# sagescherrytree/Project3-CUDA-Path-Tracer-2025

Measured on AMD Instinct MI355X. Metric: Mpaths/s (rays x bounces / s), 800x800 cornell depth 8, higher is better.
Workload: dtype f32; 1 GPU; cornell.json 800x800 depth 8, stream compaction on, sort off (BASELINE configs[1]); pipeline=fused, frames_per_pass=128, parallelism=single GPU

## Files before the change

### project3-cuda-path-tracer-2025_amd/csrc/pt_runtime.hip

```cpp
#include <dlfcn.h>
#include <hip/hip_runtime.h>
#include <hip/hip_ext.h>
#include <rccl/rccl.h>

#include <algorithm>
#include <cmath>
#include <condition_variable>
#include <mutex>
#include <thread>
#include <cstdarg>
#include <cstdlib>
#include <cstdio>
#include <cstring>
#include <string>
#include <vector>

#include "pt/pathtrace_abi.h"
#include "pt/pt_denoise.h"
#include "pt/pt_naive_mesh.h"
#include "pt_kernels.h"
#include "pt_denoise_kernels.h"
#include "pt_naive_mesh_kernels.h"
#include "trav_tree.h"

// ... 273 lines not shown
    }
    if (lds_geoms) stage_geoms(sc, s_dyn);
    PT_HOOK(STAGE_EXTRA, lds_geoms, sc, s_dyn);
    if (TIMING && active) {
        __builtin_amdgcn_s_waitcnt(0);
        uint64_t t = sec_clock();
        sec_add(SEC_LOAD, t - tc);
        sec_add(SEC_N_WAVES, 1);
        sec_add_lanes(SEC_N_LANES, p.rb > 0 ? 1 : 0);
    }
    bool live = active && p.rb > 0;
    constexpr bool MG = (VAR & VAR_MAT_GROUP) != 0;
    Hit h;
    if (MG) h = Hit{-1.f, mk(0.f, 0.f, 0.f), 0, -1, 0.f, 0.f};
    bool queued = false;
    float qt = 0.f;
    int qw = -1;
    f3 qs = mk(0.f, 0.f, 0.f);
    if (REDIST && lds_geoms) {
        if (VAR & VAR_BLOCK_REDIST)
            block_intersect<TIMING>(sc, s_geoms, live, p.o, p.d, reinterpret_cast<BlockLds*>(s_wave_isect - (tid >> 6)),
                                    qt, qw, qs);
        else
            wave_intersect<TIMING>(sc, s_geoms, live, p.o, p.d, s_wave_isect, qt, qw, qs);
    } else if (SPLIT && live) {
        prim_intersect_q<TIMING, FIRST && !TIMING>(sc, s_geoms, p.o, p.d, qt, qw, qs);
    }
    if (live) {
        if (SPLIT) {
            queued = bvh_root_needed(sc, p.o, p.d, qt);
            if (!queued) h = finish_hit<false>(sc, p.o, p.d, s_stack + tid, qt, qw, qs);
        } else if (REDIST && lds_geoms) {
            h = finish_hit<HAS_BVH, BVH_FAST>(sc, p.o, p.d, s_stack + tid, qt, qw, qs);
            PT_HOOK(DUP_HIT, HAS_BVH, BVH_FAST, sc, p.o, p.d, s_stack + tid, qt, qw, qs);
        } else {
            h = lds_geoms ? intersect_scene_q<HAS_BVH, TIMING, BVH_FAST, FIRST>(sc, s_geoms, p.o, p.d, s_stack + tid)
                          : intersect_scene<HAS_BVH, BVH_FAST>(sc, p.o, p.d, s_stack + tid);
        }
        if (!MG && !queued) {
            uint64_t ts = TIMING ? sec_clock() : 0;
            PT_HOOK(DUP_SHADE, (VAR & VAR_NO_TEX) == 0, sc, p, h, iter);
            shade_path<(VAR & VAR_NO_TEX) == 0>(sc, p, h, iter + p.slot, [&]() { return hit_attr(sc, h); });
            if (TIMING) {
                tc = sec_clock();
                sec_add(SEC_SHADE, tc - ts);
            }
        }
    }
    if (MG) {
        if (SPLIT) {
            int qi, unused;
            block_append<false>(queued, &ctl->qcnt[bounce][blockIdx.x & (NSEG - 1)][0], false, nullptr, qi, unused);
            qi += (blockIdx.x & (NSEG - 1)) * q.stride;
            if (queued) {
                queue_put(q, qi, p, qt, qw, qs);
                active = false;
                live = false;
                queued = false;
            }
        }
        const int key = live ? (h.t > 0.0f ? h.mat : 0) : MG_KEYS - 1;
        MatGroupLds* mg = reinterpret_cast<MatGroupLds*>(s_wave_isect - (tid >> 6));
        group_by_material<HAS_BVH, false>(key, mg, active, live, queued, p, h, qt, qw, qs);
        if (live) shade_path<(VAR & VAR_NO_TEX) == 0>(sc, p, h, iter + p.slot, [&]() { return hit_attr(sc, h); });
    }
    if (TIMING && active) tc = sec_clock();
    const bool surv = active && !queued && p.rb > 0;
    if (active && !queued && !surv) gather_into_image(image, sc, to_plane, p);
    const int lane = tid & 63;
    const int seg = blockIdx.x & (NSEG - 1);
    if (VAR & VAR_WAVE_ATOMIC) {
        const uint64_t m = __ballot(surv);
        if (m != 0) {
            int base = 0;
            if (lane == 0) base = atomicAdd(&ctl->cnt[bounce + 1][seg][0], __popcll(m));
            base = __shfl(base, 0);
            if (surv) store_path(out, seg * seg_stride + base + mbcnt(m), p);
        }
        if (!SPLIT) return;
        const uint64_t mq = __ballot(queued);
        if (mq != 0) {
            int base = 0;
            if (lane == 0) base = atomicAdd(&ctl->qcnt[bounce][seg][0], __popcll(mq));
            base = __shfl(base, 0);
            if (queued) {
                const int k = seg * q.stride + base + mbcnt(mq);
                queue_put(q, k, p, qt, qw, qs);
            }
        }
        return;
    }
    int si, qi;
    block_append<SPLIT>(surv, &ctl->cnt[bounce + 1][seg][0], queued, &ctl->qcnt[bounce][seg][0], si, qi);
    if (surv) store_path(out, seg * seg_stride + si, p);
    qi += seg * q.stride;
    if (SPLIT && queued) queue_put(q, qi, p, qt, qw, qs);
    if (TIMING && active) sec_add(SEC_STORE, sec_clock() - tc);
}

template <int VAR>
__global__ __launch_bounds__(BLOCK) void k_tail(SceneDev sc, PathBuf in, FrameCtl* ctl, float* __restrict__ image,
                                               int bounce, int seg_stride, int depth) {
    extern __shared__ float4 s_dyn[];
    __shared__ int s_cnt[BLOCK / 64];
    const int iter = ctl->iter;
    const bool to_plane = ctl->batch > 1 || ctl->plane != 0;
    int segoff[NSEG + 1];
    segoff[0] = 0;
#pragma unroll
    for (int s = 0; s < NSEG; ++s) segoff[s + 1] = segoff[s] + ctl->cnt[bounce][s][0];
    const int n = segoff[NSEG];
    const int block_start = blockIdx.x * BLOCK;
    if (block_start >= n) return;
    const int tid = threadIdx.x, lane = tid & 63;
    DevGeomHot* s_geoms = reinterpret_cast<DevGeomHot*>(s_dyn);
    BlockLds* s_block = reinterpret_cast<BlockLds*>(s_dyn + lds_geom_f4(sc));
    const int gid = block_start + tid;
    const bool active = gid < n;
    PathReg p;
    p.rb = 0;
    if (active) {
        int sl = 0;
#pragma unroll
        for (int k = 1; k < NSEG; ++k) sl += (gid >= segoff[k]) ? 1 : 0;
        int sofs = 0;
#pragma unroll
        for (int k = 1; k < NSEG; ++k) sofs = (sl == k) ? segoff[k] : sofs;
        p = load_path(in, sl * seg_stride + (gid - sofs));
    }
    stage_geoms(sc, s_dyn);
    const int seg = blockIdx.x & (NSEG - 1);
    for (int b = bounce; b < depth; ++b) {
        const bool live = active && p.rb > 0;
        float qt = 0.f;
        int qw = -1;
        f3 qs = mk(0.f, 0.f, 0.f);
        block_intersect<false>(sc, s_geoms, live, p.o, p.d, s_block, qt, qw, qs);
        if (live) {
            const Hit h = finish_hit<false>(sc, p.o, p.d, nullptr, qt, qw, qs);
            shade_path<(VAR & VAR_NO_TEX) == 0>(sc, p, h, iter + p.slot, [&]() { return hit_attr(sc, h); });
            if (p.rb <= 0) gather_into_image(image, sc, to_plane, p);
        }
        const bool surv = live && p.rb > 0;
        const uint64_t m = __ballot(surv);
        if (lane == 0) s_cnt[tid >> 6] = __popcll(m);
        __syncthreads();
        int tot = 0;
#pragma unroll
        for (int i = 0; i < BLOCK / 64; ++i) tot += s_cnt[i];
        if (tid == 0 && tot) atomicAdd(&ctl->cnt[b + 1][seg][0], tot);
        __syncthreads();
        if (tot == 0) break;
    }
}

#ifndef BVH_WAVES
#define BVH_WAVES 7
#endif

template <int VAR>
PT_DEV void bvh_finish_path(const SceneDev& sc, const QueueBuf& q, int qs, int iter, PathReg& p, const TravState& st) {
    float u = 0.f, v = 0.f;
    int tri = -1;
    const float tb = trav_result(st, u, v, tri);
    const float4 c = q.C[qs], d = q.D[qs];
    p.pix = __float_as_int(q.A[qs].w);
    p.rb = __float_as_int(q.B[qs].w);
    p.c = mk(c.x, c.y, c.z);
    const int cw = __float_as_int(c.w);
    p.slot = cw & 255;
    const int win = (cw >> 8) - 1;
    const Hit h = make_hit(sc, p.d, d.x, win, mk(d.y, d.z, d.w), tb, u, v, tri, sc.hot4);
    shade_path<(VAR & VAR_NO_TEX) == 0>(sc, p, h, iter + p.slot, [&]() { return hit_attr(sc, h); });
}
template <bool COUNT>
PT_DEV void bvh_count_ray(const TravState& st, float t_prim, int n_nodes) {
    if (COUNT) {
        sec_add_lanes(SEC_N_BVH_RAYS, 1);
        const bool hit = st.btri != 0x7fffffff && st.t_hit < t_prim;
        sec_add_lanes(SEC_N_BVH_HITS, hit ? 1 : 0);
        sec_add_lanes(SEC_N_MISS_NODES, hit ? 0 : n_nodes);
    }
}

PT_DEV bool tail_put(const TailBuf& t, int* ctr, int seg, int qs, const TravState& st, const int* s_stack) {
    const uint64_t m = __ballot(1);
    const int lead = __builtin_ctzll(m);
    int base = 0;
    if ((int)(threadIdx.x & 63) == lead) base = atomicAdd(ctr, __popcll(m));
    const int slot = __builtin_amdgcn_readlane(base, lead) + mbcnt(m);
    if (slot >= t.stride) return false;
    const int e = seg * t.stride + slot;
    t.node[e] = make_int2(qs, trav_saved_node(st));
    t.hit[e] = trav_saved_hit(st);
    for (int i = 0; i < min(st.sp, t.depth); ++i) t.stack[(size_t)i * t.cap + e] = s_stack[i * BLOCK];
    atomicAdd(ctr + 2, 1);
    atomicAdd(ctr + 3, st.sp);
    return true;
}

template <int VAR, bool QUAD>
__global__ __launch_bounds__(BLOCK, BVH_WAVES) void k_bvh_bounce(SceneDev sc, QueueBuf q, TailBuf tail, int defer,
                                                                 PathBuf out, FrameCtl* ctl, float* __restrict__ image,
                                                                 int bounce, int seg_stride) {
    extern __shared__ float4 s_dyn[];
    int segoff[NSEG + 1];
    segoff[0] = 0;
#pragma unroll
    for (int s = 0; s < NSEG; ++s) segoff[s + 1] = segoff[s] + ctl->qcnt[bounce][s][0];
    const int n = segoff[NSEG];
    const int block_start = blockIdx.x * BLOCK;
    if (block_start >= n) return;
    int* s_stack = reinterpret_cast<int*>(s_dyn);
    const int iter = ctl->iter;
    const bool to_plane = ctl->batch > 1 || ctl->plane != 0;
    const int tid = threadIdx.x;
    const int gid = block_start + tid;
    const int seg = blockIdx.x & (NSEG - 1);
    const bool active = gid < n;
    bool handed = false;
    const int qs = active ? segment_slot(segoff, gid, block_start, q.stride) : 0;
    PathReg p;
    p.rb = 0;
    if (active) {
        const float4 a = q.A[qs], b = q.B[qs];
        const float t_prim = q.D[qs].x;
        p.o = mk(a.x, a.y, a.z);
        p.d = mk(b.x, b.y, b.z);
        constexpr bool CNT = (VAR & VAR_SECTION_TIMING) != 0;
        int n_nodes = 0, n_tris = 0;
        TravState st;
        trav_begin(sc, st, p.o, p.d, t_prim);
        st.qs = qs;
        if (CNT) sec_add_lanes(SEC_N_ROOT_CULLED, st.cur < 0 ? 1 : 0);
        for (int d = defer;; d = 0) {
            trav_run<CNT, QUAD>(sc, st, s_stack + tid, d, n_nodes, n_tris);
            if (st.cur < 0) break;
            if (tail_put(tail, &ctl->qcnt[bounce][seg][1], seg, qs, st, s_stack + tid)) {
                handed = true;
                break;
            }
        }
        if (CNT) {
            sec_add_lanes(SEC_N_NODES, n_nodes);
            sec_add_lanes(SEC_N_TRIS, n_tris);
        }
        if (!handed) {
            bvh_count_ray<CNT>(st, t_prim, n_nodes);
            bvh_finish_path<VAR>(sc, q, qs, iter, p, st);
        }
    }
    const bool surv = active && !handed && p.rb > 0;
    if (active && !handed && !surv) gather_into_image(image, sc, to_plane, p);
    int si, unused;
    block_append<false>(surv, &ctl->cnt[bounce + 1][seg][0], false, nullptr, si, unused);
    if (surv) store_path(out, seg * seg_stride + si, p);
}

template <int VAR, bool QUAD>
__global__ __launch_bounds__(BLOCK, BVH_WAVES) void k_bvh_tail_trav(SceneDev sc, QueueBuf q, TailBuf t, FrameCtl* ctl,
                                                                    int bounce, int refill) {
    extern __shared__ float4 s_dyn[];
    int* s_stack = reinterpret_cast<int*>(s_dyn) + threadIdx.x;
    const int seg = blockIdx.x & (NSEG - 1);
    const int n = min(ctl->qcnt[bounce][seg][1], t.stride);
    if (n == 0) return;
    int next = 0;
    constexpr bool CNT = (VAR & VAR_SECTION_TIMING) != 0;
    int e = -1, qs = 0, n_nodes = 0, n_tris = 0, sp0 = 0;
    bool hit0 = false;
    TravState st;
    st.cur = -1;
    while (true) {
        const uint64_t idle = __ballot(e < 0);
        const int n_idle = __popcll(idle);
        if (next < n && (n_idle >= refill || n_idle == 64)) {
            const int lead = __builtin_ctzll(idle);
            int b0 = 0;
            if ((int)(threadIdx.x & 63) == lead) b0 = atomicAdd(&ctl->qcnt[bounce][seg][2], n_idle);
            next = __builtin_amdgcn_readlane(b0, lead);
            if (e < 0) {
                const int k = next + mbcnt(idle);
                if (k < n) {
                    e = seg * t.stride + k;
                    const int2 nd = t.node[e];
                    qs = nd.x;
                    const float4 a = q.A[qs], b = q.B[qs];
                    trav_resume(st, mk(a.x, a.y, a.z), mk(b.x, b.y, b.z), t.hit[e], nd.y, qs);
                    for (int i = 0; i < min(st.sp, sc.stack_lds); ++i) s_stack[i * BLOCK] = t.stack[(size_t)i * t.cap + e];
                    n_nodes = n_tris = 0;
                    if (CNT) {
                        sp0 = st.sp;
                        hit0 = st.btri != 0x7fffffff;
                    }
                }
            }
            next += n_idle;
        }
        const int lanes = __popcll(__ballot(e >= 0));
        if (lanes == 0) break;
        if (e >= 0) {
            if (CNT) {
                sec_add(SEC_N_BVH_WITERS, 1);
                sec_add(SEC_TAIL_LANES_HIST + (lanes - 1) / 4, 1);
            }
            trav_step<CNT, QUAD>(sc, st, s_stack, n_nodes, n_tris);
// ... 245 lines not shown
    __shared__ int h[MAXMAT];
    const int n = *n_ptr;
    const int tile = blockIdx.x, base = tile * STILE;
    for (int i = threadIdx.x; i < nkeys; i += BLOCK) h[i] = 0;
    __syncthreads();
    if (base < n) {
        for (int k = 0; k < STILE / BLOCK; ++k) {
            int idx = base + k * BLOCK + threadIdx.x;
            if (idx < n) atomicAdd(&h[keys[idx]], 1);
        }
    }
    __syncthreads();
    for (int i = threadIdx.x; i < nkeys; i += BLOCK) tile_hist[(size_t)tile * nkeys + i] = h[i];
}

__global__ __launch_bounds__(SCAN_THREADS) void k_sort_scan(int* tile_hist, const int* n_ptr, int nkeys) {
    __shared__ int s_part[SCAN_THREADS];
    const int n = *n_ptr;
    const int ntiles = (n + STILE - 1) / STILE;
    const int total = ntiles * nkeys;
    const int per = (total + SCAN_THREADS - 1) / SCAN_THREADS;
    const int tid = threadIdx.x;
    const int lo = min(total, tid * per), hi = min(total, lo + per);
    const int key0 = ntiles ? lo / ntiles : 0, t0 = lo - key0 * ntiles;
    int sum = 0;
    for (int f = lo, key = key0, t = t0; f < hi; ++f) {
        sum += tile_hist[(size_t)t * nkeys + key];
        if (++t == ntiles) { t = 0; ++key; }
    }
    s_part[tid] = sum;
    __syncthreads();
    for (int off = 1; off < SCAN_THREADS; off <<= 1) {
        const int v = tid >= off ? s_part[tid - off] : 0;
        __syncthreads();
        s_part[tid] += v;
        __syncthreads();
    }
    int run = tid ? s_part[tid - 1] : 0;
    for (int f = lo, key = key0, t = t0; f < hi; ++f) {
        const size_t at = (size_t)t * nkeys + key;
        const int c = tile_hist[at];
        tile_hist[at] = run;
        run += c;
        if (++t == ntiles) { t = 0; ++key; }
    }
}

__global__ __launch_bounds__(BLOCK) void k_sort_scatter(const int* __restrict__ keys, const int* n_ptr, int nkeys,
                                                        int key_bits, const int* tile_off, int* perm) {
    __shared__ int run[MAXMAT];
    __shared__ int wcnt[BLOCK / 64][MAXMAT];
    const int n = *n_ptr;
    const int tile = blockIdx.x, base = tile * STILE;
    if (base >= n) return;
    const int tid = threadIdx.x, w = tid >> 6;
    for (int i = tid; i < nkeys; i += BLOCK) run[i] = 0;
    __syncthreads();
    for (int k = 0; k < STILE / BLOCK; ++k) {
        int idx = base + k * BLOCK + tid;
        bool valid = idx < n;
        int key = valid ? keys[idx] : 0;
        uint64_t peers = __ballot(valid);
        for (int b = 0; b < key_bits; ++b) {
            uint64_t bb = __ballot(valid && ((key >> b) & 1));
            peers &= ((key >> b) & 1) ? bb : ~bb;
        }
        for (int i = tid; i < (BLOCK / 64) * MAXMAT; i += BLOCK) (&wcnt[0][0])[i] = 0;
        __syncthreads();
        if (valid && mbcnt(peers) == 0) wcnt[w][key] = __popcll(peers);
        __syncthreads();
        if (valid) {
            int r = run[key] + mbcnt(peers);
            for (int ww = 0; ww < w; ++ww) r += wcnt[ww][key];
            perm[tile_off[(size_t)tile * nkeys + key] + r] = idx;
        }
        __syncthreads();
        for (int key2 = tid; key2 < nkeys; key2 += BLOCK) {
            int s = 0;
            for (int ww = 0; ww < BLOCK / 64; ++ww) s += wcnt[ww][key2];
            run[key2] += s;
        }
        __syncthreads();
    }
}

__global__ void k_to_pbo(const float* __restrict__ image, pt_uchar4* pbo, int n, int iter) {
    int i = blockIdx.x * BLOCK + threadIdx.x;
    if (i >= n) return;
    int c[3];
#pragma unroll
    for (int k = 0; k < 3; ++k) {
        double d = (double)(image[3 * (size_t)i + k] / (float)iter) * 255.0;
        int v = (d != d) ? 0 : (d >= 2147483647.0 ? 2147483647 : (d <= -2147483648.0 ? (-2147483647 - 1) : (int)d));
        c[k] = v < 0 ? 0 : (v > 255 ? 255 : v);
    }
    pt_uchar4 o;
    o.x = (uint8_t)c[0];
    o.y = (uint8_t)c[1];
    o.z = (uint8_t)c[2];
    o.w = 0;
    pbo[i] = o;
}

__global__ void k_rng(const int* iid, int m, int n, float* out) {
    int i = blockIdx.x * blockDim.x + threadIdx.x;
    if (i >= m) return;
    Rng r = rng_make(iid[3 * i], iid[3 * i + 1], iid[3 * i + 2]);
    for (int k = 0; k < n; ++k) out[(size_t)i * n + k] = u01(r);
}

namespace {

thread_local std::string g_err;

int fail(int code, const char* fmt, ...) {
    char buf[512];
    va_list ap;
    va_start(ap, fmt);
    vsnprintf(buf, sizeof buf, fmt, ap);
    va_end(ap);
    g_err = buf;
    return code;
}

#define RC(x)                      \
    do {                           \
        int rc_ = (x);             \
        if (rc_ != PT_OK) return rc_; \
    } while (0)
#define HIPCHK(expr)                                                                              \
    do {                                                                                          \
        hipError_t e_ = (expr);                                                                   \
        if (e_ != hipSuccess)                                                                     \
            return fail(PT_E_HIP, "%s:%d: %s: %s", __FILE__, __LINE__, #expr, hipGetErrorString(e_)); \
    } while (0)

template <class T>
int dalloc(T** p, size_t n) {
    *p = nullptr;
    if (n == 0) return PT_OK;
    HIPCHK(hipMalloc((void**)p, n * sizeof(T)));
    return PT_OK;
}

constexpr int MAXF = 256;
constexpr int64_t AUTO_BATCH_PATHS = 84000000;

struct Tuning {
    size_t bounce_lds_pad = 0, bvh_lds_pad = 0;
    bool sections_skip_camera = false;
    bool tail_off = false;
    bool tail_any_batch = false;
    int tail_from = 0;
    int64_t auto_paths = 0;
    bool f1_graph = false;
    bool multi_f1_direct = false;
    int bvh_tail_lanes = -1;
    int bvh_tail_chunks = 0;
    int tail_refill = 16;
    int tail_trav_blocks = 224;
    int tail_shade_blocks = 512;
    bool combine_force_staged = false;
    bool bvh_tree_ref = false;
    bool bvh_tree_info = false;
    int bvh_max_height = -1;
    int bvh_quad = 1;
    int bvh_stack_lds = 0;
    int bvh_bfs_levels = 12;
    int grid = -1;
    bool speculate = true;
    int band_copy = -1;
};
Tuning read_tuning() {
    auto num = [](const char* name, long dflt) {
        const char* e = getenv(name);
        return e && *e ? atol(e) : dflt;
    };
    Tuning t;
    t.bounce_lds_pad = (size_t)std::max(0L, num("PT_BOUNCE_LDS_PAD", 0));
    t.bvh_lds_pad = (size_t)std::max(0L, num("PT_BVH_LDS_PAD", 0));
    t.sections_skip_camera = getenv("PT_SECTIONS_SKIP_CAMERA") != nullptr;
    t.tail_off = num("PT_TAIL", 1) == 0;
    t.tail_any_batch = num("PT_TAIL_BATCH", 0) != 0;
    t.tail_from = (int)num("PT_TAIL_FROM", 0);
    t.auto_paths = num("PT_AUTO_PATHS", 0);
    t.f1_graph = num("PT_F1_GRAPH", 0) != 0;
    t.multi_f1_direct = num("PT_MULTI_F1_DIRECT", 0) != 0;
    t.bvh_tail_lanes = (int)std::min(56L, std::max(-1L, num("PT_BVH_TAIL_LANES", -1)));
    t.bvh_tail_chunks = (int)std::max(0L, num("PT_BVH_TAIL_CHUNKS", 0));
    t.tail_refill = (int)std::max(1L, std::min(64L, num("PT_BVH_TAIL_REFILL", 16)));
    t.tail_trav_blocks = (int)std::max(1L, num("PT_BVH_TAIL_TRAV_BLOCKS", 224));
    t.tail_shade_blocks = (int)std::max(0L, num("PT_BVH_TAIL_SHADE_BLOCKS", 512));
    t.combine_force_staged = num("PT_COMBINE_FORCE_STAGED", 0) != 0;
    const char* tree = getenv("PT_BVH_TREE");
    t.bvh_tree_ref = tree && strcmp(tree, "ref") == 0;
    t.bvh_tree_info = getenv("PT_BVH_TREE_INFO") != nullptr;
    t.bvh_bfs_levels = (int)std::max(0L, num("PT_BVH_BFS_LEVELS", 12));
    t.bvh_max_height = (int)std::max(-1L, num("PT_BVH_MAX_HEIGHT", -1));
    t.bvh_quad = num("PT_BVH_QUAD", 1) != 0 ? 1 : 0;
    t.bvh_stack_lds = (int)std::max(0L, num("PT_BVH_STACK_LDS", 0));
    t.grid = (int)num("PT_GRID", -1);
    t.speculate = num("PT_SPECULATE", 1) != 0;
    t.band_copy = (int)std::max(-1L, std::min(1L, num("PT_BAND_COPY", -1)));
    return t;
}

struct State {
    bool inited = false;
    Tuning tune;
    pt_options opts{};
    int device = 0;
    hipStream_t stream = nullptr;
    SceneDev sc{};
    int width = 0, height = 0, pixels_total = 0, local_pixels = 0;
    int seg_stride = 0, capacity = 0;
    int alloc_frames = 0;
    bool staged_alloc = false;
    int num_tex = 0;
    bool has_bvh = false;
    int stack_depth = 0;
    int pair_depth = 0;
    size_t bvh_lds = 0;
    DevGeom* d_geoms = nullptr;
    DevCull* d_cull = nullptr;
    DevMaterial* d_mats = nullptr;
    float4* d_node_aux = nullptr;
    DevNode* d_nodes = nullptr;
    DevTriHot* d_hot = nullptr;
    DevPair* d_pairs = nullptr;
    float4* d_quads = nullptr;
    DevTriHot* d_hot4 = nullptr;
    float4* d_leaf9 = nullptr;
    DevTriCold* d_cold = nullptr;
    bool naive = false;
    DevTriHot* d_naive_hot = nullptr;
    float4* d_path[2][3] = {{nullptr, nullptr, nullptr}, {nullptr, nullptr, nullptr}};
    float4* d_hit_nt = nullptr;
    int* d_hit_mat = nullptr;
    float4* d_hit_uvd0 = nullptr;
    float4* d_hit_uvd1 = nullptr;
    uint32_t* d_texels = nullptr;
    int4* d_texinfo = nullptr;
    int* d_alive = nullptr;
    int* d_perm = nullptr;
    int* d_tile_hist = nullptr;
    int* d_tile_cnt = nullptr;
    int* d_tile_off = nullptr;
    float* d_image = nullptr;
    FrameCtl* d_ctl = nullptr;
    float* d_contrib = nullptr;
    unsigned long long* d_grid = nullptr;
    int batch = 1;
    bool split = false;
    bool no_tex = false;
    QueueBuf queue{};
    TailBuf tail{};
    int tail_lanes = 0;
    int tail_refill = 16, tail_trav_blocks = 224, tail_shade_blocks = 512;
    int tail_depth = 0;
    hipGraph_t graph[MAXF + 1] = {};
    hipGraphExec_t graph_exec[MAXF + 1] = {};
    int last_iter = 0;
    int dev_iter = 0;
    int ctl_rows = 1;
    int frames_done = 0;
    int32_t* traced_depth = nullptr;
    int* h_cnt = nullptr;
    hipStream_t spec_stream = nullptr;
    hipEvent_t spec_ev_in = nullptr;
    hipEvent_t spec_ev_done = nullptr;
    FrameCtl* d_ctl_spec = nullptr;
    float* d_spec_plane = nullptr;
    float* d_spec_sum[2] = {nullptr, nullptr};
    int spec_sum_idx = 0;
    hipStream_t copy_stream = nullptr;
    hipStream_t band_stream = nullptr;
    hipEvent_t band_ready = nullptr;
    hipGraph_t spec_graph = nullptr;
    hipGraphExec_t spec_exec = nullptr;
    int spec_iter = 0;
    int64_t spec_launched = 0, spec_adopted = 0;
    int spec_dev_iter = 0;
    int key_bits = 1;
    bool multi = false;
    float4* d_gbuf[3] = {nullptr, nullptr, nullptr};
    float4* d_dn_color[2] = {nullptr, nullptr};
    bool gbuf_valid = false;
    hipEvent_t dn_ev[PT_DENOISE_MAX_LEVELS + 3] = {};
    float dn_capture_ms = 0.f, dn_ms = 0.f, dn_level_ms[PT_DENOISE_MAX_LEVELS] = {};
};
State g_primary;
State* gp = &g_primary;
int ensure_frames(int frames);

hipError_t smemset(void* p, int v, size_t n) {
    hipError_t e = hipMemsetAsync(p, v, n, gp->stream);
    return e != hipSuccess ? e : hipStreamSynchronize(gp->stream);
}
hipError_t smemcpy(void* dst, const void* src, size_t n, hipMemcpyKind kind) {
    hipError_t e = hipMemcpyAsync(dst, src, n, kind, gp->stream);
    return e != hipSuccess ? e : hipStreamSynchronize(gp->stream);
}

PathBuf pathbuf(int i) { return PathBuf{gp->d_path[i][0], gp->d_path[i][1], gp->d_path[i][2]}; }

int ctl_reset() {
    const hipError_t e = smemset(gp->d_ctl, 0, sizeof(FrameCtl));
    if (e != hipSuccess) return fail(PT_E_HIP, "FrameCtl reset: %s", hipGetErrorString(e));
    gp->dev_iter = 0;
    return PT_OK;
}

struct ProfRec {
    int kind;
    hipEvent_t start, stop;
};
constexpr unsigned PROF_EVENT_FLAGS = hipEventDisableSystemFence;
std::vector<ProfRec>* g_prof = nullptr;
std::vector<hipEvent_t> g_prof_pool;
size_t g_prof_next = 0;

hipEvent_t prof_event() {
    if (g_prof_next < g_prof_pool.size()) return g_prof_pool[g_prof_next++];
    hipEvent_t e = nullptr;
    (void)hipEventCreateWithFlags(&e, PROF_EVENT_FLAGS);
    g_prof_pool.push_back(e);
    g_prof_next = g_prof_pool.size();
    return e;
}

template <class K, class... A>
void launch(int kind, K kernel, dim3 grid, dim3 block, uint32_t lds, A... args) {
    if (g_prof) {
        ProfRec r{kind, prof_event(), prof_event()};
        hipExtLaunchKernelGGL(kernel, grid, block, lds, gp->stream, r.start, r.stop, 0, args...);
        g_prof->push_back(r);
    } else {
        hipLaunchKernelGGL(kernel, grid, block, lds, gp->stream, args...);
    }
}
int nblocks(int n) { return (n + BLOCK - 1) / BLOCK; }

int spec_worker_idle();
void release_graph() {
    if (gp->spec_exec) {
        (void)spec_worker_idle();
        (void)hipStreamSynchronize(gp->spec_stream);
        (void)hipGraphExecDestroy(gp->spec_exec);
    }
    if (gp->spec_graph) (void)hipGraphDestroy(gp->spec_graph);
    gp->spec_exec = nullptr;
    gp->spec_graph = nullptr;
    for (int f = 0; f <= MAXF; ++f) {
        if (gp->graph_exec[f]) (void)hipGraphExecDestroy(gp->graph_exec[f]);
        if (gp->graph[f]) (void)hipGraphDestroy(gp->graph[f]);
        gp->graph_exec[f] = nullptr;
        gp->graph[f] = nullptr;
    }
}

size_t geom_table_lds() {
    return (sizeof(DevGeomHot) + (gp->sc.grid ? sizeof(DevCull) : 0)) * (size_t)gp->sc.num_geoms;
}

const int* staged_count(int b) { return &gp->d_ctl->cnt[b][0][0]; }

template <bool FIRST, bool HAS_BVH, int VAR>
void launch_bounce_t(dim3 grid, PathBuf in, PathBuf out, int b) {
    constexpr bool SPLIT = HAS_BVH && (VAR & VAR_BVH_SPLIT);
    const bool lds = (VAR & (VAR_CAND_QUEUE | VAR_WAVE_REDIST)) && gp->sc.num_geoms <= LDS_GEOMS;
    const size_t geom_lds = lds ? geom_table_lds() : 0;
    const size_t redist_lds = (VAR & VAR_WAVE_REDIST) && lds
                                  ? ((VAR & VAR_BLOCK_REDIST) ? sizeof(BlockLds) : sizeof(WaveLds) * (BLOCK / 64))
                                  : 0;
    const size_t stack_lds = HAS_BVH && !SPLIT ? gp->bvh_lds : 0;
    const size_t xchg_lds = (VAR & VAR_MAT_GROUP) ? std::max(redist_lds, mat_group_lds(HAS_BVH, false)) : redist_lds;
    const size_t bounce_pad = gp->tune.bounce_lds_pad;
    launch(100 + b, k_bounce<FIRST, HAS_BVH, VAR>, grid, dim3(BLOCK), geom_lds + stack_lds + xchg_lds + bounce_pad, gp->sc,
           in, out, gp->d_ctl, gp->d_image, b, gp->seg_stride, gp->queue);
    const size_t lds_pad = gp->tune.bvh_lds_pad;
    if (SPLIT) {
        const size_t stack_bytes = (size_t)gp->sc.stack_lds * BLOCK * sizeof(int);
        if (gp->tail_lanes > 0 && gp->sc.stack_lds > gp->tail_depth) gp->tail_lanes = 0;
        if (gp->sc.quads)
            launch(200 + b, k_bvh_bounce<VAR, true>, grid, dim3(BLOCK), stack_bytes + lds_pad, gp->sc, gp->queue,
                   gp->tail, gp->tail_lanes, out, gp->d_ctl, gp->d_image, b, gp->seg_stride);
        else
            launch(200 + b, k_bvh_bounce<VAR, false>, grid, dim3(BLOCK), stack_bytes + lds_pad, gp->sc, gp->queue,
                   gp->tail, gp->tail_lanes, out, gp->d_ctl, gp->d_image, b, gp->seg_stride);
        if (gp->tail_lanes > 0) {
            if (gp->sc.quads)
                launch(400 + b, k_bvh_tail_trav<VAR, true>, dim3(NSEG * gp->tail_trav_blocks), dim3(BLOCK), stack_bytes,
                       gp->sc, gp->queue, gp->tail, gp->d_ctl, b, gp->tail_refill);
            else
                launch(400 + b, k_bvh_tail_trav<VAR, false>, dim3(NSEG * gp->tail_trav_blocks), dim3(BLOCK), stack_bytes,
                       gp->sc, gp->queue, gp->tail, gp->d_ctl, b, gp->tail_refill);
            const int per_seg = gp->tail_shade_blocks > 0 ? std::min(gp->tail_shade_blocks, nblocks(gp->tail.stride))
                                                          : nblocks(gp->tail.stride);
            launch(400 + b, k_bvh_tail_shade<VAR>, dim3(NSEG * per_seg), dim3(BLOCK), 0, gp->sc,
                   gp->queue, gp->tail, out, gp->d_ctl, gp->d_image, b, gp->seg_stride);
        }
    }
}
template <bool FIRST, bool HAS_BVH>
void launch_bounce_v(int var, dim3 grid, PathBuf in, PathBuf out, int b) {
    switch (var) {
#ifdef PT_VAR_PROBE
        case 154: launch_bounce_t<FIRST, HAS_BVH, 154>(grid, in, out, b); break;
        case 186: launch_bounce_t<FIRST, HAS_BVH, 186>(grid, in, out, b); break;
#else
        case 0: launch_bounce_t<FIRST, HAS_BVH, 0>(grid, in, out, b); break;
        case 1: launch_bounce_t<FIRST, HAS_BVH, 1>(grid, in, out, b); break;
        case 2: launch_bounce_t<FIRST, HAS_BVH, 2>(grid, in, out, b); break;
        case 6: launch_bounce_t<FIRST, HAS_BVH, 6>(grid, in, out, b); break;
        case 10: launch_bounce_t<FIRST, HAS_BVH, 10>(grid, in, out, b); break;
        case 18: launch_bounce_t<FIRST, HAS_BVH, 18>(grid, in, out, b); break;
        case 26: launch_bounce_t<FIRST, HAS_BVH, 26>(grid, in, out, b); break;
        case 22: launch_bounce_t<FIRST, HAS_BVH, 22>(grid, in, out, b); break;
        case 50: launch_bounce_t<FIRST, HAS_BVH, 50>(grid, in, out, b); break;
        case 58: launch_bounce_t<FIRST, HAS_BVH, 58>(grid, in, out, b); break;
        case 54: launch_bounce_t<FIRST, HAS_BVH, 54>(grid, in, out, b); break;
        case 30: launch_bounce_t<FIRST, HAS_BVH, 30>(grid, in, out, b); break;
        case 154: launch_bounce_t<FIRST, HAS_BVH, 154>(grid, in, out, b); break;
        case 186: launch_bounce_t<FIRST, HAS_BVH, 186>(grid, in, out, b); break;
        case 190: launch_bounce_t<FIRST, HAS_BVH, 190>(grid, in, out, b); break;
        case 158: launch_bounce_t<FIRST, HAS_BVH, 158>(grid, in, out, b); break;
        case 666: launch_bounce_t<FIRST, HAS_BVH, 666>(grid, in, out, b); break;
        case 530: launch_bounce_t<FIRST, HAS_BVH, 530>(grid, in, out, b); break;
        case 698: launch_bounce_t<FIRST, HAS_BVH, 698>(grid, in, out, b); break;
        case 562: launch_bounce_t<FIRST, HAS_BVH, 562>(grid, in, out, b); break;
#endif
        case 1024 + 18: launch_bounce_t<FIRST, HAS_BVH, 1024 + 18>(grid, in, out, b); break;
        case 1024 + 22: launch_bounce_t<FIRST, HAS_BVH, 1024 + 22>(grid, in, out, b); break;
        case 1024 + 50: launch_bounce_t<FIRST, HAS_BVH, 1024 + 50>(grid, in, out, b); break;
        case 1024 + 54: launch_bounce_t<FIRST, HAS_BVH, 1024 + 54>(grid, in, out, b); break;
        case 1024 + 154: launch_bounce_t<FIRST, HAS_BVH, 1024 + 154>(grid, in, out, b); break;
        case 1024 + 158: launch_bounce_t<FIRST, HAS_BVH, 1024 + 158>(grid, in, out, b); break;
        case 1024 + 186: launch_bounce_t<FIRST, HAS_BVH, 1024 + 186>(grid, in, out, b); break;
        case 1024 + 190: launch_bounce_t<FIRST, HAS_BVH, 1024 + 190>(grid, in, out, b); break;
#ifndef PT_VAR_PROBE
        case 1024 + 530: launch_bounce_t<FIRST, HAS_BVH, 1024 + 530>(grid, in, out, b); break;
        case 1024 + 562: launch_bounce_t<FIRST, HAS_BVH, 1024 + 562>(grid, in, out, b); break;
        case 1024 + 666: launch_bounce_t<FIRST, HAS_BVH, 1024 + 666>(grid, in, out, b); break;
        case 1024 + 698: launch_bounce_t<FIRST, HAS_BVH, 1024 + 698>(grid, in, out, b); break;
#endif
        default: launch_bounce_t<FIRST, HAS_BVH, 3>(grid, in, out, b); break;
    }
}
bool variant_compiled(int v);
int effective_variant(bool first, int var) {
    var &= ~(VAR_BVH_NODES | VAR_NO_TEX);
    if (first) var &= ~(VAR_WAVE_REDIST | VAR_BLOCK_REDIST);
    if (first && gp->tune.sections_skip_camera) var &= ~VAR_SECTION_TIMING;
    if (!gp->split) var &= ~VAR_BVH_SPLIT;
    if (gp->no_tex && variant_compiled(var | VAR_NO_TEX)) var |= VAR_NO_TEX;
    return var;
}
bool variant_compiled(int v) {
    static const int k[] = {0, 1, 2, 6, 10, 18, 22, 26, 30, 50, 54, 58, 154, 158, 186, 190, 530, 562, 666, 698};
    static const int kt[] = {18, 22, 50, 54, 154, 158, 186, 190, 530, 562, 666, 698};
    const int* b = (v & VAR_NO_TEX) ? kt : k;
    const int n = (v & VAR_NO_TEX) ? (int)(sizeof kt / sizeof kt[0]) : (int)(sizeof k / sizeof k[0]);
    for (int i = 0; i < n; ++i)
        if (b[i] == (v & ~VAR_NO_TEX)) return true;
    return false;
}
void launch_bounce(bool first, bool bvh, int var, dim3 grid, PathBuf in, PathBuf out, int b) {
    var = effective_variant(first, var);
    if (first) {
        if (bvh) launch_bounce_v<true, true>(var, grid, in, out, b);
        else launch_bounce_v<true, false>(var, grid, in, out, b);
    } else {
        if (bvh) launch_bounce_v<false, true>(var, grid, in, out, b);
        else launch_bounce_v<false, false>(var, grid, in, out, b);
    }
}

template <int CITEMS>
void launch_compact(PathBuf pi, PathBuf po, const int* n_in, int* n_out, int npaths) {
    constexpr int CTILE = BLOCK * CITEMS;
    const int ntiles = (npaths + CTILE - 1) / CTILE;
    launch(5, k_compact_count<CITEMS>, dim3(ntiles), dim3(BLOCK), 0, (const int*)gp->d_alive, n_in, gp->d_tile_cnt);
    launch(5, k_compact_scan, dim3(1), dim3(SCAN_THREADS), 0, (const int*)gp->d_tile_cnt, n_in, gp->d_tile_off, n_out,
           CTILE);
    launch(3, k_compact_scatter<CITEMS>, dim3(ntiles), dim3(BLOCK), 0, (const float4*)pi.A, (const float4*)pi.B,
           (const float4*)pi.C, po.A, po.B, po.C, (const int*)gp->d_alive, n_in, (const int*)gp->d_tile_off);
}

int tail_from(int batch) {
    const int depth = gp->sc.trace_depth;
    const bool lds = gp->sc.num_geoms <= LDS_GEOMS;
    if (gp->tune.tail_off || (batch != 1 && !gp->tune.tail_any_batch) || gp->has_bvh || !lds || depth < 3 ||
        (effective_variant(false, gp->opts.variant) & ~VAR_NO_TEX) !=
            (VAR_CAND_QUEUE | VAR_WAVE_REDIST | VAR_BVH_FAST | VAR_BLOCK_REDIST))
        return 0;
    const int from = gp->tune.tail_from;
    return std::min(depth - 1, std::max(1, from > 0 ? from : depth / 2));
}

int enqueue_pass_body(int batch) {
    const int depth = gp->sc.trace_depth;
    const int npaths = gp->local_pixels * batch;
    const int nb = nblocks(npaths);
    const int nbounces = std::max(1, depth);
    if (gp->opts.pipeline == PT_PIPELINE_FUSED) {
        const int t = tail_from(batch);
        for (int b = 0; b < (t ? t : nbounces); ++b) {
            PathBuf in = pathbuf(b & 1), out = pathbuf((b + 1) & 1);
            launch_bounce(b == 0, gp->has_bvh, gp->opts.variant & ~VAR_BVH_NODES, dim3(nb), in, out, b);
            HIPCHK(hipGetLastError());
        }
        if (t) {
            constexpr int V = VAR_CAND_QUEUE | VAR_WAVE_REDIST | VAR_BVH_FAST | VAR_BLOCK_REDIST;
            const size_t lds = geom_table_lds() + sizeof(BlockLds);
            if (gp->no_tex)
                launch(300 + t, k_tail<V | VAR_NO_TEX>, dim3(nb), dim3(BLOCK), lds, gp->sc, pathbuf(t & 1), gp->d_ctl,
                       gp->d_image, t, gp->seg_stride, depth);
            else
                launch(300 + t, k_tail<V>, dim3(nb), dim3(BLOCK), lds, gp->sc, pathbuf(t & 1), gp->d_ctl, gp->d_image, t,
                       gp->seg_stride, depth);
            HIPCHK(hipGetLastError());
        }
        return PT_OK;
    }
    launch(0, k_camera, dim3(nb), dim3(BLOCK), 0, gp->sc, pathbuf(0), gp->d_ctl);
    HIPCHK(hipGetLastError());
    const int stiles = (npaths + STILE - 1) / STILE;
    int cur = 0;
    for (int b = 0; b < nbounces; ++b) {
        const int* n_in = gp->opts.stream_compaction ? staged_count(b) : staged_count(0);
        HitBuf hits{gp->d_hit_nt, gp->d_hit_mat, gp->d_hit_uvd0, gp->d_hit_uvd1};
        if (gp->has_bvh && (gp->opts.variant & VAR_BVH_FAST))
            launch(1, k_intersect<true, true>, dim3(nb), dim3(BLOCK), gp->bvh_lds, gp->sc, pathbuf(cur), hits, n_in);
        else if (gp->has_bvh)
            launch(1, k_intersect<true, false>, dim3(nb), dim3(BLOCK), gp->bvh_lds, gp->sc, pathbuf(cur), hits, n_in);
        else
            launch(1, k_intersect<false, false>, dim3(nb), dim3(BLOCK), 0, gp->sc, pathbuf(cur), hits, n_in);
        if (gp->naive && gp->sc.num_tris > 0)
            launch(7, k_naive_mesh, dim3(nb), dim3(BLOCK), 0, gp->sc, (const DevTriHot*)gp->d_naive_hot, gp->sc.num_tris,
                   pathbuf(cur), hits.nt, hits.mat, hits.uvd0, hits.uvd1, n_in);
        HIPCHK(hipGetLastError());
        const int* perm = nullptr;
        if (gp->opts.material_sort) {
            const int nk = std::max(1, gp->sc.num_mats);
            launch(4, k_sort_hist, dim3(stiles), dim3(BLOCK), 0, (const int*)gp->d_hit_mat, n_in, nk, gp->d_tile_hist);
            launch(4, k_sort_scan, dim3(1), dim3(SCAN_THREADS), 0, gp->d_tile_hist, n_in, nk);
            launch(4, k_sort_scatter, dim3(stiles), dim3(BLOCK), 0, (const int*)gp->d_hit_mat, n_in, nk, gp->key_bits,
                   (const int*)gp->d_tile_hist, gp->d_perm);
            HIPCHK(hipGetLastError());
            perm = gp->d_perm;
        }
        launch(2, k_shade, dim3(nb), dim3(BLOCK), 0, gp->sc, pathbuf(cur), hits, perm, n_in, (const FrameCtl*)gp->d_ctl,
               0, gp->d_image, gp->opts.stream_compaction ? gp->d_alive : (int*)nullptr);
        HIPCHK(hipGetLastError());
        if (gp->opts.stream_compaction) {
            PathBuf pi = pathbuf(cur), po = pathbuf(cur ^ 1);
            int* n_out = &gp->d_ctl->cnt[b + 1][0][0];
            launch_compact<CITEMS>(pi, po, n_in, n_out, npaths);
            HIPCHK(hipGetLastError());
            cur ^= 1;
        }
    }
    return PT_OK;
}

int enqueue_pass(int set_iter, int batch, int plane = 0) {
    gp->ctl_rows = std::max(gp->ctl_rows, std::min(MAXB + 1, gp->sc.trace_depth + 1));
    launch(-1, k_frame_begin, dim3(1), dim3(256), 0, gp->d_ctl, set_iter, gp->local_pixels, batch, gp->ctl_rows, plane);
    HIPCHK(hipGetLastError());
    RC(enqueue_pass_body(batch));
    if (batch > 1) {
        launch(6, k_combine, dim3(nblocks(gp->local_pixels)), dim3(BLOCK), 0, gp->sc, (const FrameCtl*)gp->d_ctl,
               gp->d_image);
        HIPCHK(hipGetLastError());
    }
    return PT_OK;
}

int build_graph(int batch) {
    HIPCHK(hipStreamBeginCapture(gp->stream, hipStreamCaptureModeThreadLocal));
    int rc = enqueue_pass(0, batch);
    hipGraph_t gr = nullptr;
    hipError_t e = hipStreamEndCapture(gp->stream, &gr);
    if (rc != PT_OK) return rc;
    HIPCHK(e);
    gp->graph[batch] = gr;
    HIPCHK(hipGraphInstantiate(&gp->graph_exec[batch], gr, nullptr, nullptr, 0));
    return PT_OK;
}

int run_pass(int iter, int batch) {
    RC(ensure_frames(batch));
    if (gp->opts.use_graph && (batch > 1 || gp->tune.f1_graph || (gp->multi && !gp->tune.multi_f1_direct))) {
        if (!gp->graph_exec[batch]) RC(build_graph(batch));
        if (gp->dev_iter != iter - 1) HIPCHK(hipMemsetD32Async((hipDeviceptr_t)&gp->d_ctl->iter, iter - 1, 1, gp->stream));
        HIPCHK(hipGraphLaunch(gp->graph_exec[batch], gp->stream));
    } else {
        RC(enqueue_pass(iter, batch));
    }
    gp->dev_iter = iter;
    gp->last_iter = iter + batch - 1;
    gp->frames_done += batch;
    return PT_OK;
}
int run_frame(int iter) { return run_pass(iter, 1); }

struct SpecTask {
    int device = 0;
    hipStream_t stream = nullptr;
    hipEvent_t ev_in = nullptr, ev_done = nullptr;
    hipGraphExec_t exec = nullptr;
    int* iter_ptr = nullptr;
    int preset = -1;
    const float* image = nullptr;
    const float* plane = nullptr;
    float* sum = nullptr;
    int nf = 0;
};
struct SpecLauncher {
    std::thread th;
    std::mutex mu;
    std::condition_variable cv;
    bool task = false, busy = false, stop = false;
    hipError_t err = hipSuccess;
    SpecTask tasks[PT_MAX_DEVICES];
    int ntasks = 0;

    static hipError_t launch_one(const SpecTask& t) {
        hipError_t e = hipSetDevice(t.device);
        if (e == hipSuccess) e = hipStreamWaitEvent(t.stream, t.ev_in, 0);
        if (e == hipSuccess && t.preset >= 0) e = hipMemsetD32Async((hipDeviceptr_t)t.iter_ptr, t.preset, 1, t.stream);
        if (e == hipSuccess) e = hipGraphLaunch(t.exec, t.stream);
        if (e == hipSuccess) {
            hipLaunchKernelGGL(k_spec_sum, dim3(nblocks((t.nf + 3) / 4)), dim3(BLOCK), 0, t.stream, t.image, t.plane,
                               t.sum, t.nf);
            e = hipGetLastError();
        }
        if (e == hipSuccess) e = hipEventRecord(t.ev_done, t.stream);
        return e;
    }
    void run() {
        std::unique_lock<std::mutex> lk(mu);
        for (;;) {
            cv.wait(lk, [&] { return task || stop; });
            if (stop) return;
            task = false;
            SpecTask ts[PT_MAX_DEVICES];
            const int n = ntasks;
            for (int i = 0; i < n; ++i) ts[i] = tasks[i];
            lk.unlock();
            hipError_t e = hipSuccess;
            for (int i = 0; i < n && e == hipSuccess; ++i) e = launch_one(ts[i]);
            lk.lock();
            if (e != hipSuccess) err = e;
            busy = false;
            cv.notify_all();
        }
    }
    void post(const SpecTask* t, int n) {
        std::lock_guard<std::mutex> lk(mu);
// ... 2473 lines not shown
```

Baseline: 36570 Mpaths/s.

## Fuse camera bounce and first secondary bounce into a single head kernel

Adds a k_head kernel that generates camera rays, intersects and shades the primary hit, then does the second bounce in the same block and writes survivors with block_append. The fused pipeline skips the first two bounce launches and starts its loop at bounce 2, and the tail start is clamped to at least 2. This removes one kernel launch plus the write and reread of the full path buffer between bounce 0 and bounce 1. The cost is a larger kernel with more register pressure, and no compaction between the two fused bounces, so blocks keep dead lanes through the second intersection.

```diff
diff --git a/project3-cuda-path-tracer-2025_amd/csrc/pt_runtime.hip b/project3-cuda-path-tracer-2025_amd/csrc/pt_runtime.hip
--- a/project3-cuda-path-tracer-2025_amd/csrc/pt_runtime.hip
+++ b/project3-cuda-path-tracer-2025_amd/csrc/pt_runtime.hip
@@ -449,6 +449,61 @@
         __syncthreads();
         if (tot == 0) break;
     }
+}
+
+template <int VAR>
+__global__ __launch_bounds__(BLOCK) void k_head(SceneDev sc, PathBuf out, FrameCtl* ctl, float* __restrict__ image,
+                                               int seg_stride) {
+    extern __shared__ float4 s_dyn[];
+    const int iter = ctl->iter;
+    const bool to_plane = ctl->batch > 1 || ctl->plane != 0;
+    const int n = ctl->cnt[0][0][0];
+    const int block_start = blockIdx.x * BLOCK;
+    if (block_start >= n) return;
+    const int tid = threadIdx.x, lane = tid & 63;
+    DevGeomHot* s_geoms = reinterpret_cast<DevGeomHot*>(s_dyn);
+    BlockLds* s_block = reinterpret_cast<BlockLds*>(s_dyn + lds_geom_f4(sc));
+    int* s_cnt = reinterpret_cast<int*>(s_block->rt);
+    const int gid = block_start + tid;
+    const bool active = gid < n;
+    PathReg p;
+    p.rb = 0;
+    if (active) {
+        const int slot = gid / sc.shard.local_pixels;
+        p = camera_ray(sc.cam, iter + slot, sc.trace_depth, shard_pixel(sc, gid - slot * sc.shard.local_pixels));
+        p.slot = slot;
+    }
+    stage_geoms(sc, s_dyn);
+    const int seg = blockIdx.x & (NSEG - 1);
+    if (active && p.rb > 0) {
+        const Hit h = intersect_scene_q<false, false, true, true>(sc, s_geoms, p.o, p.d, nullptr);
+        shade_path<(VAR & VAR_NO_TEX) == 0>(sc, p, h, iter + p.slot, [&]() { return hit_attr(sc, h); });
+    }
+    bool live = active && p.rb > 0;
+    if (active && !live) gather_into_image(image, sc, to_plane, p);
+    {
+        const uint64_t m = __ballot(live);
+        if (lane == 0) s_cnt[tid >> 6] = __popcll(m);
+        __syncthreads();
+        int tot = 0;
+#pragma unroll
+        for (int i = 0; i < BLOCK / 64; ++i) tot += s_cnt[i];
+        if (tid == 0 && tot) atomicAdd(&ctl->cnt[1][seg][0], tot);
+        if (tot == 0) return;
+    }
+    float qt = 0.f;
+    int qw = -1;
+    f3 qs = mk(0.f, 0.f, 0.f);
+    block_intersect<false>(sc, s_geoms, live, p.o, p.d, s_block, qt, qw, qs);
+    if (live) {
+        const Hit h = finish_hit<false>(sc, p.o, p.d, nullptr, qt, qw, qs);
+        shade_path<(VAR & VAR_NO_TEX) == 0>(sc, p, h, iter + p.slot, [&]() { return hit_attr(sc, h); });
+        if (p.rb <= 0) gather_into_image(image, sc, to_plane, p);
+    }
+    const bool surv = live && p.rb > 0;
+    int si, unused;
+    block_append<false>(surv, &ctl->cnt[2][seg][0], false, nullptr, si, unused);
+    if (surv) store_path(out, seg * seg_stride + si, p);
 }
 
 #ifndef BVH_WAVES
@@ -1000,6 +1055,7 @@
     bool tail_off = false;
     bool tail_any_batch = false;
     int tail_from = 0;
+    bool head_fuse = true;
     int64_t auto_paths = 0;
     bool f1_graph = false;
     bool multi_f1_direct = false;
@@ -1031,6 +1087,7 @@
     t.tail_off = num("PT_TAIL", 1) == 0;
     t.tail_any_batch = num("PT_TAIL_BATCH", 0) != 0;
     t.tail_from = (int)num("PT_TAIL_FROM", 0);
+    t.head_fuse = num("PT_HEAD_FUSE", 1) != 0;
     t.auto_paths = num("PT_AUTO_PATHS", 0);
     t.f1_graph = num("PT_F1_GRAPH", 0) != 0;
     t.multi_f1_direct = num("PT_MULTI_F1_DIRECT", 0) != 0;
@@ -1335,6 +1392,14 @@
            (const float4*)pi.C, po.A, po.B, po.C, (const int*)gp->d_alive, n_in, (const int*)gp->d_tile_off);
 }
 
+bool head_fused() {
+    constexpr int V0 = VAR_CAND_QUEUE | VAR_BVH_FAST;
+    constexpr int V1 = VAR_CAND_QUEUE | VAR_WAVE_REDIST | VAR_BVH_FAST | VAR_BLOCK_REDIST;
+    const int var = gp->opts.variant & ~VAR_BVH_NODES;
+    return gp->tune.head_fuse && gp->opts.pipeline == PT_PIPELINE_FUSED && !gp->has_bvh &&
+           gp->sc.num_geoms <= LDS_GEOMS && gp->sc.trace_depth >= 2 &&
+           (effective_variant(true, var) & ~VAR_NO_TEX) == V0 && (effective_variant(false, var) & ~VAR_NO_TEX) == V1;
+}
 int tail_from(int batch) {
     const int depth = gp->sc.trace_depth;
     const bool lds = gp->sc.num_geoms <= LDS_GEOMS;
@@ -1343,7 +1408,7 @@
             (VAR_CAND_QUEUE | VAR_WAVE_REDIST | VAR_BVH_FAST | VAR_BLOCK_REDIST))
         return 0;
     const int from = gp->tune.tail_from;
-    return std::min(depth - 1, std::max(1, from > 0 ? from : depth / 2));
+    return std::min(depth - 1, std::max(head_fused() ? 2 : 1, from > 0 ? from : depth / 2));
 }
 
 int enqueue_pass_body(int batch) {
@@ -1353,7 +1418,18 @@
     const int nbounces = std::max(1, depth);
     if (gp->opts.pipeline == PT_PIPELINE_FUSED) {
         const int t = tail_from(batch);
-        for (int b = 0; b < (t ? t : nbounces); ++b) {
+        const bool head = head_fused();
+        if (head) {
+            const size_t lds = geom_table_lds() + sizeof(BlockLds) + gp->tune.bounce_lds_pad;
+            if (gp->no_tex)
+                launch(100, k_head<VAR_NO_TEX>, dim3(nb), dim3(BLOCK), lds, gp->sc, pathbuf(0), gp->d_ctl, gp->d_image,
+                       gp->seg_stride);
+            else
+                launch(100, k_head<0>, dim3(nb), dim3(BLOCK), lds, gp->sc, pathbuf(0), gp->d_ctl, gp->d_image,
+                       gp->seg_stride);
+            HIPCHK(hipGetLastError());
+        }
+        for (int b = head ? 2 : 0; b < (t ? t : nbounces); ++b) {
             PathBuf in = pathbuf(b & 1), out = pathbuf((b + 1) & 1);
             launch_bounce(b == 0, gp->has_bvh, gp->opts.variant & ~VAR_BVH_NODES, dim3(nb), in, out, b);
             HIPCHK(hipGetLastError());
```

After: 38380 Mpaths/s, median of 6. 1.05x the previous value.
